# OpenDriveLab/MTGS

Measured on AMD Instinct MI355X. Metric: rendered Mpix/s (fwd+bwd) @ 2M Gaussians 1920x1080, higher is better.
Workload: dtype f32

## Files before the change

mtgs_amd/csrc/bin3.hip:

```cpp
#include "common.hpp"
#include "tile_rect.hpp"
#include "devsize.hpp"
#include "raster_rec.hpp"

namespace {

using mtgs_os::SizeRef;

constexpr int B3_BLOCK = 256;
constexpr int MAX_BINS = 32768;

struct Item { uint32_t rank, span; };
constexpr int SPAN_BITS = 12;
constexpr int MAX_ROWS = 4096;

struct RowGeom {
    int row0, h, tile0, w;
    int y0, x0;
    float mx, my, ca, cb, cc, s2max;
};
template <bool TIGHT>
__device__ __forceinline__ RowGeom row_geom(const float *__restrict__ recs, const int32_t *__restrict__ vis_ids, int64_t rank,
                                            int64_t N, int C, float ts, int tw, int th) {
    const float4 *rec = reinterpret_cast<const float4 *>(recs + rank * REC_FLOATS);
    const float4 r0 = rec[0], r1 = rec[1];
    const Rect q = tile_rect(r0.x, r0.y, __float_as_int(r1.w), ts, tw, th);
    const int cam = C == 1 ? 0 : (int)((uint32_t)vis_ids[rank] / (uint32_t)N);
    RowGeom g;
    g.row0 = cam * th + q.y0; g.h = q.y1 - q.y0; g.w = q.x1 - q.x0;
    g.tile0 = g.row0 * tw + q.x0;
    g.y0 = q.y0; g.x0 = q.x0;
    g.mx = r0.x; g.my = r0.y; g.ca = r0.z; g.cb = r0.w; g.cc = r1.x; g.s2max = r1.z;
    if (g.w <= 0) g.h = 0;
    if (TIGHT && !(g.s2max >= 0.f)) g.h = 0;
    return g;
}
template <bool TIGHT>
__device__ __forceinline__ int row_span(const RowGeom &g, int y, int tw, int &first) {
    first = g.tile0 + y * tw;
    if (!TIGHT) return g.w;
    const float a = g.ca, b = g.cb, c = g.cc, det = a * c - b * b;
    if (!(det > 0.f && a > 0.f && c > 0.f)) return g.w;
    const float ty = (float)((g.y0 + y) * MTGS_TILE_SIZE);
    const float Y0 = ty + 0.5f - g.my, Y1 = ty + 15.5f - g.my;
    const float sm = g.s2max * 1.001f + 1e-2f;
    const float rdet = 1.0f / det, ymax = sqrtf(a * sm * rdet), X = sqrtf(sm * c * rdet);
    const float yb0 = fmaxf(Y0, -ymax), yb1 = fminf(Y1, ymax);
    if (!(yb0 <= yb1)) return 0;
    const float ra = 1.0f / a, tilt = b * X / c;
    const float dyl = fminf(fmaxf(tilt, yb0), yb1), dyr = fminf(fmaxf(-tilt, yb0), yb1);
    const float xl = (-b * dyl - sqrtf(fmaxf(a * sm - det * dyl * dyl, 0.f))) * ra - 2e-3f;
    const float xr = (-b * dyr + sqrtf(fmaxf(a * sm - det * dyr * dyr, 0.f))) * ra + 2e-3f;
    const float inv = 1.0f / (float)MTGS_TILE_SIZE;
    const float fx0 = (float)g.x0, fx1 = (float)(g.x0 + g.w);
    const int lo = (int)fminf(fmaxf(ceilf((g.mx + xl - 15.5f) * inv), fx0), fx1) - g.x0;
    const int hi = (int)fmaxf(fminf(floorf((g.mx + xr - 0.5f) * inv), fx1 - 1.f), fx0 - 1.f) - g.x0 + 1;
    first += lo;
    return hi - lo;
}

__device__ __forceinline__ bool arrive_last(uint32_t *done, int64_t active, int *s_flag) {
    __syncthreads();
    if (threadIdx.x == 0)
        *s_flag = __hip_atomic_fetch_add(done, 1u, __ATOMIC_RELAXED, __HIP_MEMORY_SCOPE_AGENT) == (uint32_t)(active - 1);
    __syncthreads();
    return *s_flag != 0;
}

constexpr int R_BLOCK = 1024;
constexpr int SERIAL_MAX = 48;

struct RowShare {
    float mx[R_BLOCK], my[R_BLOCK], ca[R_BLOCK], cb[R_BLOCK], cc[R_BLOCK], s2[R_BLOCK];
    uint32_t xy[R_BLOCK];
    uint32_t wr[R_BLOCK];
    uint32_t off[R_BLOCK + 1];
    uint32_t ws[R_BLOCK / 64];
};
template <class F>
__device__ __forceinline__ void tight_rows_walk(RowShare &S, const RowGeom &g, int h, int tw, F &&emit) {
    const int tid = threadIdx.x, lane = tid & 63, wave = tid >> 6;
    S.mx[tid] = g.mx; S.my[tid] = g.my; S.ca[tid] = g.ca; S.cb[tid] = g.cb; S.cc[tid] = g.cc; S.s2[tid] = g.s2max;
    S.xy[tid] = (uint32_t)g.x0 | ((uint32_t)g.y0 << 16);
    S.wr[tid] = (uint32_t)max(g.w - 1, 0) | ((uint32_t)g.row0 << 16);
    uint32_t inc = (uint32_t)h;
#pragma unroll
    for (int o = 1; o < 64; o <<= 1) {
        const uint32_t up = __shfl_up(inc, o, 64);
        if (lane >= o) inc += up;
    }
    if (lane == 63) S.ws[wave] = inc;
    __syncthreads();
    uint32_t base = 0;
    for (int w = 0; w < wave; ++w) base += S.ws[w];
    S.off[tid] = base + inc - (uint32_t)h;
    if (tid == R_BLOCK - 1) S.off[R_BLOCK] = base + inc;
    __syncthreads();
    const uint32_t total = S.off[R_BLOCK];
    static_assert(R_BLOCK == 1 << 10, "ten bisection steps");
    for (uint32_t idx = tid; idx < total; idx += R_BLOCK) {
        int lo = 0, hi = R_BLOCK;
#pragma unroll
        for (int it = 0; it < 10; ++it) {
            const int mid = (lo + hi) >> 1;
            if (S.off[mid] <= idx) lo = mid; else hi = mid;
        }
        const int y = (int)(idx - S.off[lo]);
        RowGeom q;
        q.mx = S.mx[lo]; q.my = S.my[lo]; q.ca = S.ca[lo]; q.cb = S.cb[lo]; q.cc = S.cc[lo]; q.s2max = S.s2[lo];
        const uint32_t xy = S.xy[lo], wr = S.wr[lo];
        q.x0 = (int)(xy & 0xffffu); q.y0 = (int)(xy >> 16); q.w = (int)(wr & 0xffffu) + 1; q.row0 = (int)(wr >> 16);
        q.tile0 = q.row0 * tw + q.x0; q.h = 0;
        int first;
        const int w = row_span<true>(q, y, tw, first);
        if (w > 0) emit(lo, q.row0 + y, first, w);
    }
}
template <bool TIGHT>
__global__ __launch_bounds__(R_BLOCK) void bin3_rows_count_kernel(const SizeRef n_vis_ref, const float *__restrict__ recs,
                                                                 const int32_t *__restrict__ vis_ids, int64_t N, int C, float ts,
                                                                 int tw, int th, int n_rows, uint32_t *__restrict__ row_count,
                                                                 uint32_t *__restrict__ rbase, uint32_t *__restrict__ done,
                                                                 uint32_t *__restrict__ row_start ) {
    __shared__ uint32_t s_row[MAX_ROWS];
    __shared__ uint32_t s_ws[R_BLOCK / 64];
    __shared__ uint16_t s_tall[R_BLOCK];
    __shared__ uint32_t s_ntall;
    __shared__ int s_last;
    const int tid = threadIdx.x, lane = tid & 63, wave = tid >> 6;
    const int64_t n_vis = mtgs_os::size_of(n_vis_ref);
    const int64_t r = (int64_t)blockIdx.x * R_BLOCK + tid;
    if ((int64_t)blockIdx.x * R_BLOCK >= n_vis) {
        if (n_vis == 0 && blockIdx.x == 0)
            for (int b = tid; b <= n_rows; b += R_BLOCK) row_start[b] = 0;
        return;
    }
    for (int b = tid; b < n_rows; b += R_BLOCK) s_row[b] = 0;
    if (tid == 0) s_ntall = 0;
    __syncthreads();
    RowGeom g = {};
    int my_rows = 0;
    if (r < n_vis) {
        g = row_geom<TIGHT>(recs, vis_ids, r, N, C, ts, tw, th);
        if (g.h <= SERIAL_MAX) {
            my_rows = g.h;
            if (!TIGHT)
                for (int y = 0; y < g.h; ++y) atomicAdd(&s_row[g.row0 + y], 1u);
        } else {
            s_tall[atomicAdd(&s_ntall, 1u)] = (uint16_t)tid;
        }
    }
    if constexpr (TIGHT) {
        __shared__ RowShare s_share;
        tight_rows_walk(s_share, g, my_rows, tw, [&](int, int bin, int, int) { atomicAdd(&s_row[bin], 1u); });
    }
    __syncthreads();
    for (uint32_t q = wave; q < s_ntall; q += R_BLOCK / 64) {
        const RowGeom g = row_geom<TIGHT>(recs, vis_ids, (int64_t)blockIdx.x * R_BLOCK + s_tall[q], N, C, ts, tw, th);
        int first;
        for (int y = lane; y < g.h; y += 64)
            if (row_span<TIGHT>(g, y, tw, first) > 0) atomicAdd(&s_row[g.row0 + y], 1u);
    }
    __syncthreads();
    for (int b = tid; b < n_rows; b += R_BLOCK) {
        const uint32_t c = s_row[b];
        if (c) rbase[(size_t)blockIdx.x * n_rows + b] = __hip_atomic_fetch_add(row_count + b, c, __ATOMIC_RELAXED, __HIP_MEMORY_SCOPE_AGENT);
    }
    if (!arrive_last(done, ceil_div64(n_vis, R_BLOCK), &s_last)) return;
    constexpr int ROWS_PER_THREAD = MAX_ROWS / R_BLOCK;
    static_assert(MAX_ROWS % R_BLOCK == 0, "whole rows per thread");
    uint32_t v[ROWS_PER_THREAD], mine = 0;
#pragma unroll
    for (int e = 0; e < ROWS_PER_THREAD; ++e) {
        const int b = tid * ROWS_PER_THREAD + e;
        v[e] = b < n_rows ? mtgs_os::ld32(row_count + b) : 0u;
        mine += v[e];
    }
    uint32_t inc = mine;
#pragma unroll
    for (int o = 1; o < 64; o <<= 1) {
        const uint32_t up = __shfl_up(inc, o, 64);
        if (lane >= o) inc += up;
    }
    if (lane == 63) s_ws[wave] = inc;
    __syncthreads();
    uint32_t run = inc - mine;
    for (int w = 0; w < wave; ++w) run += s_ws[w];
#pragma unroll
    for (int e = 0; e < ROWS_PER_THREAD; ++e) {
        const int b = tid * ROWS_PER_THREAD + e;
        if (b < n_rows) row_start[b] = run;
        run += v[e];
        if (b == n_rows - 1) row_start[n_rows] = run;
    }
}

template <bool TIGHT>
__global__ __launch_bounds__(R_BLOCK) void bin3_rows_place_kernel(const SizeRef n_vis_ref, const float *__restrict__ recs,
                                                                 const int32_t *__restrict__ vis_ids, int64_t N, int C, float ts,
                                                                 int tw, int th, int n_rows, const uint32_t *__restrict__ row_start,
                                                                 const uint32_t *__restrict__ rbase, int64_t cap_items,
                                                                 Item *__restrict__ items) {
    __shared__ uint32_t s_row[MAX_ROWS];
    __shared__ uint16_t s_tall[R_BLOCK];
    __shared__ uint32_t s_ntall;
    const int tid = threadIdx.x, lane = tid & 63, wave = tid >> 6;
    const int64_t n_vis = mtgs_os::size_of(n_vis_ref);
    if ((int64_t)blockIdx.x * R_BLOCK >= n_vis) return;
    for (int b = tid; b < n_rows; b += R_BLOCK) s_row[b] = row_start[b] + rbase[(size_t)blockIdx.x * n_rows + b];
    if (tid == 0) s_ntall = 0;
    __syncthreads();
    const int64_t r = (int64_t)blockIdx.x * R_BLOCK + tid;
    RowGeom g = {};
    int my_rows = 0;
    if (r < n_vis) {
        g = row_geom<TIGHT>(recs, vis_ids, r, N, C, ts, tw, th);
        if (g.h <= SERIAL_MAX) {
            my_rows = g.h;
            if (!TIGHT)
                for (int y = 0; y < g.h; ++y) {
                    const int64_t pos = atomicAdd(&s_row[g.row0 + y], 1u);
                    if (pos < cap_items) items[pos] = Item{(uint32_t)r, ((uint32_t)(g.tile0 + y * tw) << SPAN_BITS) | (uint32_t)(g.w - 1)};
                }
        } else {
            s_tall[atomicAdd(&s_ntall, 1u)] = (uint16_t)tid;
        }
    }
    if constexpr (TIGHT) {
        __shared__ RowShare s_share;
        const int64_t r0 = (int64_t)blockIdx.x * R_BLOCK;
        tight_rows_walk(s_share, g, my_rows, tw, [&](int owner, int bin, int first, int w) {
            const int64_t pos = atomicAdd(&s_row[bin], 1u);
            if (pos < cap_items) items[pos] = Item{(uint32_t)(r0 + owner), ((uint32_t)first << SPAN_BITS) | (uint32_t)(w - 1)};
        });
    }
    __syncthreads();
    for (uint32_t q = wave; q < s_ntall; q += R_BLOCK / 64) {
        const int64_t rq = (int64_t)blockIdx.x * R_BLOCK + s_tall[q];
        const RowGeom g = row_geom<TIGHT>(recs, vis_ids, rq, N, C, ts, tw, th);
        for (int y = lane; y < g.h; y += 64) {
            int first;
            const int w = row_span<TIGHT>(g, y, tw, first);
            if (w <= 0) continue;
            const int64_t pos = atomicAdd(&s_row[g.row0 + y], 1u);
            if (pos < cap_items) items[pos] = Item{(uint32_t)rq, ((uint32_t)first << SPAN_BITS) | (uint32_t)(w - 1)};
        }
    }
}

constexpr int SM_LONG_BUCKET = 255;
constexpr int T_THREADS = 1024, T_ITEMS = 2, T_TILE = T_THREADS * T_ITEMS, SCHED_BUCKETS = 1024;
struct TileRange { int lo, hi; };
__device__ __forceinline__ TileRange tile_range(const Item *__restrict__ items, int64_t base, int64_t n_items, int tw) {
    const int64_t last = min(n_items, base + T_TILE) - 1;
    const int first_tile = (int)(items[base].span >> SPAN_BITS), last_tile = (int)(items[last].span >> SPAN_BITS);
    return TileRange{(first_tile / tw) * tw, (last_tile / tw + 1) * tw};
}

__global__ __launch_bounds__(T_THREADS) void bin3_tiles_count_kernel(
    const uint32_t *__restrict__ n_items_ptr, int64_t cap_items, const Item *__restrict__ items, int tw, int n_bins,
    int64_t cap_M, uint32_t *__restrict__ bins , uint32_t *__restrict__ done ,
    int32_t *__restrict__ offsets , int32_t *__restrict__ order ,
    uint32_t *__restrict__ n_long ) {
    extern __shared__ uint32_t s_bins[];
    __shared__ uint32_t s_aux[SCHED_BUCKETS];
    __shared__ uint32_t s_ws[T_THREADS / 64];
    __shared__ uint16_t s_wide[T_TILE];
    __shared__ uint32_t s_nwide;
    __shared__ int s_last;
    const int tid = threadIdx.x, lane = tid & 63, wave = tid >> 6;
    const int64_t n_items = min((int64_t)*n_items_ptr, cap_items);
    if ((int64_t)blockIdx.x * T_TILE >= n_items) {
        if (n_items == 0 && blockIdx.x == 0) {
            for (int b = tid; b <= n_bins; b += T_THREADS) offsets[b] = 0;
            for (int b = tid; b < n_bins; b += T_THREADS) order[b] = b;
            if (tid == 0) *n_long = 0;
        }
        return;
    }
    for (int64_t base = (int64_t)blockIdx.x * T_TILE; base < n_items; base += (int64_t)gridDim.x * T_TILE) {
        const TileRange tr = tile_range(items, base, n_items, tw);
        for (int b = tr.lo + tid; b < tr.hi; b += T_THREADS) s_bins[b] = 0;
        if (tid == 0) s_nwide = 0;
        __syncthreads();
#pragma unroll
        for (int e = 0; e < T_ITEMS; ++e) {
            const int64_t i = base + e * T_THREADS + tid;
            if (i < n_items) {
                const Item it = items[i];
                const int t0 = (int)(it.span >> SPAN_BITS), w = (int)(it.span & ((1u << SPAN_BITS) - 1)) + 1;
                if (w <= SERIAL_MAX) {
                    for (int x = 0; x < w; ++x) atomicAdd(&s_bins[t0 + x], 1u);
                } else {
                    s_wide[atomicAdd(&s_nwide, 1u)] = (uint16_t)(e * T_THREADS + tid);
                }
            }
        }
        __syncthreads();
        for (uint32_t q = wave; q < s_nwide; q += T_THREADS / 64) {
            const Item it = items[base + s_wide[q]];
            const int t0 = (int)(it.span >> SPAN_BITS), w = (int)(it.span & ((1u << SPAN_BITS) - 1)) + 1;
            for (int x = lane; x < w; x += 64) atomicAdd(&s_bins[t0 + x], 1u);
        }
        __syncthreads();
        for (int b = tr.lo + tid; b < tr.hi; b += T_THREADS) {
            const uint32_t c = s_bins[b];
            if (c) {
                const uint32_t before = __hip_atomic_fetch_add(bins + b, c, __ATOMIC_RELAXED, __HIP_MEMORY_SCOPE_AGENT);
                asm volatile("" ::"v"(before));
            }
        }
        __syncthreads();
    }
    if (!arrive_last(done, min((int64_t)gridDim.x, ceil_div64(n_items, T_TILE)), &s_last)) return;
    for (int b = tid; b < n_bins; b += T_THREADS) s_bins[b] = mtgs_os::ld32(bins + b);
    __syncthreads();
    const int per = (n_bins + T_THREADS - 1) / T_THREADS;
    const int b0 = tid * per, b1 = min(n_bins, b0 + per);
    uint32_t mine = 0;
    for (int b = b0; b < b1; ++b) mine += s_bins[b];
    uint32_t inc = mine;
#pragma unroll
    for (int o = 1; o < 64; o <<= 1) {
        const uint32_t up = __shfl_up(inc, o, 64);
        if (lane >= o) inc += up;
    }
    if (lane == 63) s_ws[wave] = inc;
    __syncthreads();
    uint32_t wb = 0;
    for (int w = 0; w < wave; ++w) wb += s_ws[w];
    uint64_t run = (uint64_t)wb + inc - mine;
    const uint64_t cap = (uint64_t)cap_M;
    for (int b = b0; b < b1; ++b) {
        const uint64_t lo = run < cap ? run : cap;
        run += s_bins[b];
        const uint64_t hi = run < cap ? run : cap;
        offsets[b] = (int32_t)lo;
        s_bins[b] = (uint32_t)(hi - lo);
        if (b == n_bins - 1) offsets[n_bins] = (int32_t)hi;
    }
    s_aux[tid] = 0;
    __syncthreads();
    auto bucket_of = [&](int t) { return SCHED_BUCKETS - 1 - min((int)(s_bins[t] >> 2), SCHED_BUCKETS - 1); };
    for (int t = tid; t < n_bins; t += T_THREADS) atomicAdd(&s_aux[bucket_of(t)], 1u);
    __syncthreads();
    const uint32_t hv = s_aux[tid];
    uint32_t hinc = hv;
#pragma unroll
    for (int o = 1; o < 64; o <<= 1) {
        const uint32_t up = __shfl_up(hinc, o, 64);
        if (lane >= o) hinc += up;
    }
    if (lane == 63) s_ws[wave] = hinc;
    __syncthreads();
    uint32_t hb = 0;
    for (int w = 0; w < wave; ++w) hb += s_ws[w];
    __syncthreads();
    s_aux[tid] = hb + hinc - hv;
    __syncthreads();
    if (tid == 0) *n_long = s_aux[SCHED_BUCKETS - SM_LONG_BUCKET];
    __syncthreads();
    for (int t = tid; t < n_bins; t += T_THREADS) order[atomicAdd(&s_aux[bucket_of(t)], 1u)] = t;
}

struct TailFill {
    int mode;
    const int64_t *totals;
    int32_t *flatten_ids;
    int64_t *isect_ids;
    int64_t sentinel_key;
    int64_t *status;
    int64_t cap_vis, cap_M;
};

__global__ __launch_bounds__(T_THREADS) void bin3_tiles_place_kernel(
    const uint32_t *__restrict__ n_items_ptr, int64_t cap_items, const Item *__restrict__ items, int tw, int n_bins,
    const int32_t *__restrict__ offsets, uint32_t *__restrict__ cursor ,
    const uint64_t *__restrict__ vis_keys, uint32_t cap_keys, uint64_t *__restrict__ keys64, const TailFill tail) {
    extern __shared__ uint32_t s_bins[];
    __shared__ uint16_t s_wide[T_TILE];
    __shared__ uint32_t s_nwide;
    const int tid = threadIdx.x, lane = tid & 63, wave = tid >> 6;
    const int64_t n_items = min((int64_t)*n_items_ptr, cap_items);
    for (int64_t base = (int64_t)blockIdx.x * T_TILE; base < n_items; base += (int64_t)gridDim.x * T_TILE) {
        const TileRange tr = tile_range(items, base, n_items, tw);
        for (int b = tr.lo + tid; b < tr.hi; b += T_THREADS) s_bins[b] = 0;
        if (tid == 0) s_nwide = 0;
        __syncthreads();
        Item it[T_ITEMS];
        int t0[T_ITEMS], w[T_ITEMS];
        uint32_t depth[T_ITEMS];
#pragma unroll
        for (int e = 0; e < T_ITEMS; ++e) {
            const int64_t i = base + e * T_THREADS + tid;
            it[e] = Item{0, 0}; t0[e] = 0; w[e] = 0; depth[e] = 0;
            if (i < n_items) {
                it[e] = items[i];
                t0[e] = (int)(it[e].span >> SPAN_BITS); w[e] = (int)(it[e].span & ((1u << SPAN_BITS) - 1)) + 1;
                depth[e] = (uint32_t)vis_keys[it[e].rank];
                if (w[e] <= SERIAL_MAX) {
                    for (int x = 0; x < w[e]; ++x) atomicAdd(&s_bins[t0[e] + x], 1u);
                } else {
                    s_wide[atomicAdd(&s_nwide, 1u)] = (uint16_t)(e * T_THREADS + tid);
                    w[e] = 0;
                }
            }
        }
        __syncthreads();
        const uint32_t n_wide = s_nwide;
        for (uint32_t q = wave; q < n_wide; q += T_THREADS / 64) {
            const Item iw = items[base + s_wide[q]];
            const int tq = (int)(iw.span >> SPAN_BITS), wq = (int)(iw.span & ((1u << SPAN_BITS) - 1)) + 1;
            for (int x = lane; x < wq; x += 64) atomicAdd(&s_bins[tq + x], 1u);
        }
        __syncthreads();
        for (int b = tr.lo + tid; b < tr.hi; b += T_THREADS) {
            const uint32_t c = s_bins[b];
            if (c) s_bins[b] = (uint32_t)offsets[b] + __hip_atomic_fetch_add(cursor + b, c, __ATOMIC_RELAXED, __HIP_MEMORY_SCOPE_AGENT);
        }
        __syncthreads();
#pragma unroll
        for (int e = 0; e < T_ITEMS; ++e) {
            const uint64_t key = ((uint64_t)depth[e] << 32) | it[e].rank;
            for (int x = 0; x < w[e]; ++x) {
                const uint32_t pos = atomicAdd(&s_bins[t0[e] + x], 1u);
                if (pos < cap_keys) keys64[pos] = key;
            }
        }
        for (uint32_t q = wave; q < n_wide; q += T_THREADS / 64) {
            const Item iw = items[base + s_wide[q]];
            const int tq = (int)(iw.span >> SPAN_BITS), wq = (int)(iw.span & ((1u << SPAN_BITS) - 1)) + 1;
            const uint64_t key = ((uint64_t)(uint32_t)vis_keys[iw.rank] << 32) | iw.rank;
            for (int x = lane; x < wq; x += 64) {
                const uint32_t pos = atomicAdd(&s_bins[tq + x], 1u);
                if (pos < cap_keys) keys64[pos] = key;
            }
        }
        __syncthreads();
    }
    if (tail.status && blockIdx.x == 0 && tid == 0) {
        const int64_t packed = *tail.totals, nv = packed >> 32, m = packed & 0xFFFFFFFFll;
        tail.status[0] = nv;
        tail.status[1] = m;
        tail.status[2] = (nv > tail.cap_vis || m > tail.cap_M) ? 1 : 0;
    }
    if (tail.mode) {
        const int64_t from = offsets[n_bins];
        int64_t to = (int64_t)cap_keys;
        if (tail.mode == 2) to = min(to, (int64_t)(*tail.totals & 0xFFFFFFFFll));
        for (int64_t i = from + (int64_t)blockIdx.x * T_THREADS + tid; i < to; i += (int64_t)gridDim.x * T_THREADS) {
            tail.flatten_ids[i] = -1;
            if (tail.isect_ids) tail.isect_ids[i] = tail.sentinel_key;
        }
    }
}

struct SortEpilogue {
    int32_t *rank_ids, *flatten_ids;
    int64_t *isect_ids;
    const int32_t *vis_ids;
    uint32_t n_tiles;
    int tile_bits;
    bool single_cam;
    uint32_t rank_max;
    __device__ __forceinline__ void store(int64_t dst, uint32_t bin, uint64_t key) const {
        const int32_t rank = (int32_t)min((uint32_t)key, rank_max);
        rank_ids[dst] = rank;
        __builtin_nontemporal_store(vis_ids[rank], flatten_ids + dst);
        if (isect_ids) {
            const int64_t cam = single_cam ? 0 : bin / n_tiles, tile = single_cam ? bin : bin % n_tiles;
            __builtin_nontemporal_store((long long)((cam << (32 + tile_bits)) | (tile << 32) | (int64_t)(key >> 32)), reinterpret_cast<long long *>(isect_ids) + dst);
        }
    }
};

constexpr uint64_t KEY_INF = 0x7ff0000000000000ull;
__host__ __device__ constexpr int swz_t(int hi4) {
    return ((hi4 & 1) ? 15 : 0) ^ ((hi4 & 2) ? 11 : 0) ^ ((hi4 & 4) ? 29 : 0) ^ ((hi4 & 8) ? 17 : 0);
}
__device__ __forceinline__ int swz(int i) {
    const int t = (int)((0x1916121d040b0f00ull >> ((i >> 2) & 0x38)) & 31);
    return i ^ t ^ ((i & 256) ? 17 : 0);
}
static_assert(swz_t(1) == 0x0f && swz_t(2) == 0x0b && swz_t(3) == 0x04 && swz_t(4) == 0x1d && swz_t(5) == 0x12 &&
              swz_t(6) == 0x16 && swz_t(7) == 0x19 && swz_t(8) == 17, "packed table");
__host__ __device__ constexpr int swz_d(int d) { return d ^ swz_t((d >> 5) & 15); }
__device__ __forceinline__ void cswap(uint64_t &a, uint64_t &b) {
    const double x = __longlong_as_double((long long)a), y = __longlong_as_double((long long)b);
    double lo, hi;
    asm("v_min_f64 %0, %1, %2" : "=v"(lo) : "v"(x), "v"(y));
    asm("v_max_f64 %0, %1, %2" : "=v"(hi) : "v"(x), "v"(y));
    a = (uint64_t)__double_as_longlong(lo); b = (uint64_t)__double_as_longlong(hi);
}
template <bool WAVE> __device__ __forceinline__ void lds_sync() {
    if constexpr (WAVE) {
        __builtin_amdgcn_fence(__ATOMIC_RELEASE, "wavefront");
        __builtin_amdgcn_wave_barrier();
        __builtin_amdgcn_fence(__ATOMIC_ACQUIRE, "wavefront");
    } else {
        __syncthreads();
    }
}

template <bool WAVE, int LOGE, int STOP>
__device__ __forceinline__ void trip(uint64_t *s, int groups, int n, int nthr, int tid, int apply) {
    constexpr int E = 1 << LOGE, SLOW = STOP >> (LOGE - 1);
    if constexpr (SLOW >= 1) {
        for (int g = tid; g < groups; g += nthr) {
            const int x = ((g & ~(SLOW - 1)) << LOGE) | (g & (SLOW - 1));
            if (x >= n) continue;
            const int px = swz(x);
            uint64_t v[E];
#pragma unroll
            for (int e = 0; e < E; ++e) v[e] = s[px ^ swz_d(e * SLOW)];
#pragma unroll
            for (int bit = E >> 1; bit >= 1; bit >>= 1)
                if (apply & bit) {
#pragma unroll
                    for (int e = 0; e < E; ++e)
                        if (!(e & bit)) cswap(v[e], v[e | bit]);
                }
#pragma unroll
            for (int e = 0; e < E; ++e) s[px ^ swz_d(e * SLOW)] = v[e];
        }
        lds_sync<WAVE>();
    }
}
template <bool WAVE, int LOGE, int H>
__device__ __forceinline__ void mirror_trip(uint64_t *s, int groups, int n, int nthr, int tid) {
    constexpr int E = 1 << LOGE, HALF = E >> 1, B = H >> (LOGE - 1);
    if constexpr (B >= 1) {
        for (int g = tid; g < groups; g += nthr) {
            const int x = ((g & ~(B - 1)) << LOGE) | (g & (B - 1));
            if (x >= n) continue;
            const int low = x & (B - 1);
            const int pl = swz(x), pu = swz(x - low + H + (B - 1 - low));
            uint64_t v[E];
#pragma unroll
            for (int f = 0; f < HALF; ++f) { v[f] = s[pl ^ swz_d(f * B)]; v[HALF + f] = s[pu ^ swz_d(f * B)]; }
#pragma unroll
            for (int f = 0; f < HALF; ++f) cswap(v[f], v[E - 1 - f]);
#pragma unroll
            for (int bit = HALF >> 1; bit >= 1; bit >>= 1) {
#pragma unroll
                for (int f = 0; f < HALF; ++f)
                    if (!(f & bit)) { cswap(v[f], v[f | bit]); cswap(v[HALF + f], v[HALF + (f | bit)]); }
            }
#pragma unroll
            for (int f = 0; f < HALF; ++f) { s[pl ^ swz_d(f * B)] = v[f]; s[pu ^ swz_d(f * B)] = v[HALF + f]; }
        }
        lds_sync<WAVE>();
    }
}
#define B3_STRIDE_SWITCH(J, CALL)                                                                                   \
    switch (J) {                                                                                                     \
        case 4: CALL(4); break; case 8: CALL(8); break; case 16: CALL(16); break; case 32: CALL(32); break;          \
        case 64: CALL(64); break; case 128: CALL(128); break; case 256: CALL(256); break; case 512: CALL(512); break; \
        case 1024: CALL(1024); break; case 2048: CALL(2048); break; case 4096: CALL(4096); break;                   \
        default: CALL(8192); break;                                                                                   \
    }

template <bool WAVE, int LOGE>
__device__ __forceinline__ void level_tail(uint64_t *s, int groups, int n, int nthr, int tid, int j) {
    constexpr int E = 1 << LOGE;
    int r = 0;
    for (int q = j; q >= 1; q >>= 1) ++r;
    while (r > LOGE) {
        const int take = r - LOGE >= LOGE ? LOGE : r - LOGE;
        const int apply = ((1 << take) - 1) << (LOGE - take);
#define B3_CALL(S) trip<WAVE, LOGE, S>(s, groups, n, nthr, tid, apply)
        B3_STRIDE_SWITCH(j, B3_CALL)
#undef B3_CALL
        j >>= take;
        r -= take;
    }
    trip<WAVE, LOGE, E / 2>(s, groups, n, nthr, tid, (1 << r) - 1);
}

template <bool WAVE, int LOGE>
__device__ __forceinline__ void bitonic_sort_e(uint64_t *s, int P, int n, int nthr, int tid) {
    constexpr int E = 1 << LOGE;
    const int groups = P >> LOGE;
    for (int g = tid; g < groups; g += nthr) {
        const int x = g << LOGE;
        if (x >= n) continue;
        const int px = swz(x);
        uint64_t v[E];
#pragma unroll
        for (int e = 0; e < E; ++e) v[e] = s[px ^ e];
#pragma unroll
        for (int k = 2; k <= E; k <<= 1) {
#pragma unroll
            for (int e = 0; e < E; ++e)
                if ((e ^ (k - 1)) > e) cswap(v[e], v[e ^ (k - 1)]);
#pragma unroll
            for (int j = k >> 2; j >= 1; j >>= 1) {
#pragma unroll
                for (int e = 0; e < E; ++e)
                    if (!(e & j)) cswap(v[e], v[e | j]);
            }
        }
#pragma unroll
        for (int e = 0; e < E; ++e) s[px ^ e] = v[e];
    }
    lds_sync<WAVE>();
    for (int k = 2 * E; k <= P; k <<= 1) {
        const int h = k >> 1;
#define B3_CALL(S) mirror_trip<WAVE, LOGE, S>(s, groups, n, nthr, tid)
        B3_STRIDE_SWITCH(h, B3_CALL)
#undef B3_CALL
        if ((k >> (LOGE + 1)) >= 1) level_tail<WAVE, LOGE>(s, groups, n, nthr, tid, k >> (LOGE + 1));
    }
}
template <bool WAVE, int P16 = 1 << 30>
__device__ __forceinline__ void bitonic_sort(uint64_t *s, int P, int n, int nthr, int tid) {
    if constexpr (P16 < (1 << 30)) {
        if (P >= P16) { bitonic_sort_e<WAVE, 4>(s, P, n, nthr, tid); return; }
    }
    bitonic_sort_e<WAVE, 3>(s, P, n, nthr, tid);
}

__device__ __forceinline__ int pow2_ceil(int n) {
    int p = 8;
    while (p < n) p <<= 1;
    return p;
}

template <bool WAVE, int P16 = 1 << 30>
__device__ __forceinline__ void sort_tile_lds(uint64_t *s, const uint64_t *__restrict__ keys, int64_t o0, int L, uint32_t bin,
                                              int nthr, int tid, const SortEpilogue &epi) {
    const int P = pow2_ceil(L);
    for (int i = tid; i < P; i += nthr) s[swz(i)] = i < L ? keys[o0 + i] : KEY_INF;
    lds_sync<WAVE>();
    bitonic_sort<WAVE, P16>(s, P, L, nthr, tid);
    for (int i = tid; i < L; i += nthr) epi.store(o0 + i, bin, s[swz(i)]);
    lds_sync<WAVE>();
}

constexpr int SM_CAP = 4096, SM_WAVE_CAP = 1024, SM_TILES = 4;
constexpr int LG_THREADS = 1024, LG_CAP = 16384;
__global__ __launch_bounds__(B3_BLOCK, 4) void bin3_sort_small_kernel(const int32_t *__restrict__ offsets,
                                                                  const int32_t *__restrict__ order, int n_bins,
                                                                  const uint32_t *__restrict__ n_long_ptr, int64_t cap_M,
                                                                  const uint64_t *__restrict__ keys, const SortEpilogue epi) {
    __shared__ uint64_t s_keys[SM_CAP];
    static_assert(SM_CAP == SM_TILES * SM_WAVE_CAP, "one buffer: a long list, or four short ones");
    const int tid = threadIdx.x, wave = tid >> 6, lane = tid & 63;
    const int n_long = (int)*n_long_ptr;
    const bool together = (int)blockIdx.x < n_long;
    const int g = together ? (int)blockIdx.x : n_long + ((int)blockIdx.x - n_long) * SM_TILES + wave;
    if (g >= n_bins) return;
    const int bin = order[g];
    const int o0 = offsets[bin], L = offsets[bin + 1] - o0;
    if (L == 0 || L > SM_CAP || (int64_t)o0 + L > cap_M) return;
    if (together) sort_tile_lds<false, 4096>(s_keys, keys, o0, L, (uint32_t)bin, B3_BLOCK, tid, epi);
    else if (L <= SM_WAVE_CAP) sort_tile_lds<true, 1024>(s_keys + wave * SM_WAVE_CAP, keys, o0, L, (uint32_t)bin, 64, lane, epi);
}

__global__ __launch_bounds__(LG_THREADS) void bin3_sort_large_kernel(const int32_t *__restrict__ offsets,
                                                                    const int32_t *__restrict__ order, int n_bins, int64_t cap_M,
                                                                    uint64_t *keys, const SortEpilogue epi) {
    extern __shared__ uint64_t s_big[];
    const int tid = threadIdx.x;
    for (int g = blockIdx.x; g < n_bins; g += gridDim.x) {
        const int bin = order[g];
        const int64_t o0 = offsets[bin];
        const int L = offsets[bin + 1] - (int)o0;
        if (L <= SM_CAP) {
            if ((L >> 2) < SCHED_BUCKETS - 1) break;
            continue;
        }
        if (o0 + L > cap_M) continue;
        if (L <= LG_CAP) {
            sort_tile_lds<false>(s_big, keys, o0, L, (uint32_t)bin, LG_THREADS, tid, epi);
            continue;
        }
        uint64_t *seg = keys + o0;
        const int nch = (L + LG_CAP - 1) / LG_CAP;
        for (int c = 0; c < nch; ++c) {
            const int c0 = c * LG_CAP, n = min(LG_CAP, L - c0);
            for (int i = tid; i < LG_CAP; i += LG_THREADS) s_big[swz(i)] = i < n ? seg[c0 + i] : KEY_INF;
            __syncthreads();
            bitonic_sort<false>(s_big, LG_CAP, n, LG_THREADS, tid);
            for (int i = tid; i < n; i += LG_THREADS) seg[c0 + i] = s_big[swz(i)];
            __syncthreads();
        }
        int64_t P = LG_CAP;
        while (P < L) P <<= 1;
        for (int64_t k = 2 * LG_CAP; k <= P; k <<= 1) {
            const int64_t half = k >> 1;
            for (int64_t i = tid; i < P / 2; i += LG_THREADS) {
                const int64_t b = (i / half) * k, o = i % half, lo = b + o, hi = b + k - 1 - o;
                if (hi < L) {
                    uint64_t a = seg[lo], z = seg[hi];
                    if (a > z) { seg[lo] = z; seg[hi] = a; }
                }
            }
            __syncthreads();
            for (int64_t j = k >> 2; j >= LG_CAP; j >>= 1) {
                for (int64_t i = tid; i < P / 2; i += LG_THREADS) {
                    const int64_t lo = (i / j) * 2 * j + i % j, hi = lo + j;
                    if (hi < L) {
                        uint64_t a = seg[lo], z = seg[hi];
                        if (a > z) { seg[lo] = z; seg[hi] = a; }
                    }
                }
                __syncthreads();
            }
            for (int c = 0; c < nch; ++c) {
                const int c0 = c * LG_CAP, n = min(LG_CAP, L - c0);
                for (int i = tid; i < LG_CAP; i += LG_THREADS) s_big[swz(i)] = i < n ? seg[c0 + i] : KEY_INF;
                __syncthreads();
                level_tail<false, 3>(s_big, LG_CAP >> 3, n, LG_THREADS, tid, LG_CAP >> 1);
                for (int i = tid; i < n; i += LG_THREADS) seg[c0 + i] = s_big[swz(i)];
                __syncthreads();
            }
        }
        for (int i = tid; i < L; i += LG_THREADS) epi.store(o0 + i, (uint32_t)bin, seg[i]);
        __syncthreads();
    }
}

inline int bit_length_u32(uint32_t v) {
    int b = 0;
    while (v) { ++b; v >>= 1; }
    return b;
}

struct Bin3Workspace {
    char *control;
    size_t control_bytes;
    uint32_t *done_rows, *done_tiles, *n_long, *row_count, *bins, *cursor;
    uint32_t *row_start, *rbase;
    int32_t *order;
    Item *items;
    uint64_t *keys64;
    size_t total;
};
inline Bin3Workspace carve3(char *base, int64_t cap_vis, int64_t cap_M, int n_rows, int n_bins) {
    Bin3Workspace w;
    size_t off = 0;
    auto take = [&](size_t bytes) { char *p = base ? base + off : nullptr; off += mtgs_os::align256(bytes); return p; };
    const int64_t m = cap_M > 0 ? cap_M : 1, nv = cap_vis > 0 ? cap_vis : 1;
    w.control = base;
    char *misc = take(64);
    w.done_rows = (uint32_t *)misc; w.done_tiles = (uint32_t *)misc + 1; w.n_long = (uint32_t *)misc + 2;
    w.row_count = (uint32_t *)take((size_t)n_rows * 4);
    w.bins = (uint32_t *)take((size_t)n_bins * 4);
    w.cursor = (uint32_t *)take((size_t)n_bins * 4);
    w.control_bytes = off;
    w.row_start = (uint32_t *)take((size_t)(n_rows + 1) * 4);
    w.rbase = (uint32_t *)take((size_t)ceil_div64(nv, R_BLOCK) * n_rows * 4);
    w.order = (int32_t *)take((size_t)n_bins * 4);
    w.items = (Item *)take((size_t)m * sizeof(Item));
    w.keys64 = (uint64_t *)take((size_t)m * 8);
    w.total = off;
    return w;
}

}

extern "C" int mtgs_bin3_supported(int C, int tile_w, int tile_h, int64_t cap_M) {
    return C > 0 && tile_w > 0 && tile_h > 0 && (int64_t)C * tile_w * tile_h <= MAX_BINS && (int64_t)C * tile_h <= MAX_ROWS && tile_w <= (1 << SPAN_BITS) &&
                   cap_M < ((int64_t)1 << 30)
               ? 1 : 0;
}

extern "C" int mtgs_bin3_control_bytes(int C, int tile_w, int tile_h, size_t *bytes) {
    MTGS_REQUIRE(C > 0 && tile_w > 0 && tile_h > 0 && bytes, MTGS_EINVAL, "mtgs_bin3_control_bytes: bad arguments");
    *bytes = carve3(nullptr, 1, 1, C * tile_h, C * tile_w * tile_h).control_bytes;
    return MTGS_OK;
}

extern "C" int mtgs_bin3_workspace_bytes(int C, int tile_w, int tile_h, int64_t cap_vis, int64_t cap_M, size_t *bytes) {
    MTGS_REQUIRE(C > 0 && tile_w > 0 && tile_h > 0 && cap_vis >= 0 && cap_M >= 0 && bytes, MTGS_EINVAL,
                 "mtgs_bin3_workspace_bytes: bad arguments");
    *bytes = carve3(nullptr, cap_vis, cap_M, C * tile_h, C * tile_w * tile_h).total;
    return MTGS_OK;
}

extern "C" int mtgs_bin3_build(int C, int64_t N, int tile_size, int tile_w, int tile_h, int64_t *totals,
                               int64_t cap_vis, int64_t cap_M, const float *recs, const int32_t *vis_ids,
                               const int64_t *vis_keys, int32_t *rank_ids,
                               int32_t *flatten_ids, int64_t *isect_ids, int32_t *offsets, int32_t *tile_order, int flags,
                               void *ws, size_t ws_bytes, void *stream) {
    const int tight = flags & MTGS_BIN3_TIGHT;
    MTGS_REQUIRE((flags & ~(MTGS_BIN3_TIGHT | MTGS_BIN3_FILL_TO_M | MTGS_BIN3_FILL_TO_CAP | MTGS_BIN3_PREZEROED | MTGS_BIN3_STATUS)) == 0, MTGS_EINVAL,
                 "mtgs_bin3_build: unknown flags %d", flags);
    MTGS_REQUIRE(C > 0 && N >= 0 && tile_w > 0 && tile_h > 0 && cap_vis >= 0 && cap_M >= 0, MTGS_EINVAL, "mtgs_bin3_build: bad sizes");
    MTGS_REQUIRE(tile_size == MTGS_TILE_SIZE, MTGS_EUNSUPPORTED, "mtgs_bin3_build: tile_size=%d (only 16 is implemented)", tile_size);
    MTGS_REQUIRE(mtgs_bin3_supported(C, tile_w, tile_h, cap_M), MTGS_EUNSUPPORTED,
                 "mtgs_bin3_build: %d x %d x %d (camera, tile) pairs / %lld intersections (at most %d pairs, %d (camera, tile row) "
                 "pairs and 2^30 intersections; use mtgs_bin_build)", C, tile_w, tile_h, (long long)cap_M, MAX_BINS, MAX_ROWS);
    MTGS_REQUIRE(totals && recs && vis_ids && vis_keys && rank_ids && flatten_ids && offsets && ws, MTGS_EINVAL,
                 "mtgs_bin3_build: null pointer");
    const int n_bins = C * tile_w * tile_h, n_rows = C * tile_h;
    MTGS_REQUIRE((reinterpret_cast<uintptr_t>(ws) & 255) == 0, MTGS_EINVAL, "mtgs_bin3_build: workspace must be 256-byte aligned");
    Bin3Workspace w = carve3((char *)ws, cap_vis, cap_M, n_rows, n_bins);
    MTGS_REQUIRE(ws_bytes >= w.total, MTGS_EWORKSPACE, "mtgs_bin3_build: workspace %zu < %zu bytes", ws_bytes, w.total);
    hipStream_t st = (hipStream_t)stream;
    if (!(flags & MTGS_BIN3_PREZEROED))
        if (int rc = mtgs_zero_async(w.control, w.control_bytes, st)) return rc;
    const SizeRef n_vis_ref{totals, 1, cap_vis};
    int32_t *order = tile_order ? tile_order : w.order;
    const unsigned r_grid = (unsigned)ceil_div64(cap_vis > 0 ? cap_vis : 1, R_BLOCK);
    const unsigned t_grid = (unsigned)min((int64_t)512, ceil_div64(cap_M > 0 ? cap_M : 1, T_TILE));
    const float ts = (float)tile_size;
    if (tight) {
        bin3_rows_count_kernel<true><<<r_grid, R_BLOCK, 0, st>>>(n_vis_ref, recs, vis_ids, N, C, ts, tile_w, tile_h, n_rows, w.row_count,
                                                                w.rbase, w.done_rows, w.row_start);
        bin3_rows_place_kernel<true><<<r_grid, R_BLOCK, 0, st>>>(n_vis_ref, recs, vis_ids, N, C, ts, tile_w, tile_h, n_rows, w.row_start,
                                                                w.rbase, cap_M, w.items);
    } else {
        bin3_rows_count_kernel<false><<<r_grid, R_BLOCK, 0, st>>>(n_vis_ref, recs, vis_ids, N, C, ts, tile_w, tile_h, n_rows, w.row_count,
                                                                 w.rbase, w.done_rows, w.row_start);
        bin3_rows_place_kernel<false><<<r_grid, R_BLOCK, 0, st>>>(n_vis_ref, recs, vis_ids, N, C, ts, tile_w, tile_h, n_rows, w.row_start,
                                                                 w.rbase, cap_M, w.items);
    }
    const int tile_bits_ = bit_length_u32((uint32_t)(tile_w * tile_h));
    const TailFill tail{cap_M > 0 ? ((flags & MTGS_BIN3_FILL_TO_CAP) ? 4 : ((flags & MTGS_BIN3_FILL_TO_M) ? 2 : 0)) : 0, totals, flatten_ids, isect_ids,
                        ((int64_t)(C - 1) << (32 + tile_bits_)) | ((int64_t)(tile_w * tile_h - 1) << 32) | (int64_t)0x7f800000,
                        (flags & MTGS_BIN3_STATUS) ? totals + 1 : nullptr, cap_vis, cap_M};
    bin3_tiles_count_kernel<<<t_grid, T_THREADS, (size_t)n_bins * 4, st>>>(w.row_start + n_rows, cap_M, w.items, tile_w, n_bins,
                                                                            cap_M, w.bins, w.done_tiles, offsets, order, w.n_long);
    bin3_tiles_place_kernel<<<t_grid, T_THREADS, (size_t)n_bins * 4, st>>>(w.row_start + n_rows, cap_M, w.items, tile_w, n_bins,
                                                                            offsets, w.cursor, (const uint64_t *)vis_keys, (uint32_t)(cap_M > 0 ? cap_M : 1), w.keys64, tail);
    const SortEpilogue epi{rank_ids, flatten_ids, isect_ids, vis_ids, (uint32_t)(tile_w * tile_h),
                           bit_length_u32((uint32_t)(tile_w * tile_h)), C == 1, (uint32_t)(cap_vis > 0 ? cap_vis - 1 : 0)};
    static const bool big_lds = [] {
        return hipFuncSetAttribute((const void *)bin3_sort_large_kernel, hipFuncAttributeMaxDynamicSharedMemorySize,
                                   LG_CAP * 8) == hipSuccess &&
               hipFuncSetAttribute((const void *)bin3_tiles_place_kernel, hipFuncAttributeMaxDynamicSharedMemorySize,
                                   MAX_BINS * 4) == hipSuccess &&
               hipFuncSetAttribute((const void *)bin3_tiles_count_kernel, hipFuncAttributeMaxDynamicSharedMemorySize,
                                   MAX_BINS * 4) == hipSuccess;
    }();
    MTGS_REQUIRE(big_lds, MTGS_ELAUNCH, "mtgs_bin3_build: cannot reserve %d bytes of LDS per workgroup", LG_CAP * 8);
    bin3_sort_large_kernel<<<(unsigned)min(n_bins, 256), LG_THREADS, (size_t)LG_CAP * 8, st>>>(
        offsets, order, n_bins, cap_M, w.keys64, epi);
    bin3_sort_small_kernel<<<(unsigned)n_bins, B3_BLOCK, 0, st>>>(offsets, order, n_bins, w.n_long, cap_M, w.keys64, epi);
    MTGS_CHECK_LAUNCH("mtgs_bin3_build");
    return MTGS_OK;
}
```

Before: 2643.

## Move tile scan out of count kernel; placers compute offsets locally

The count kernel no longer elects a last-arriving block to prefix-scan all bins and build the tile schedule. Block 0 of the place kernel now builds the schedule (offsets, order, long-bin count) while the other blocks derive each bin's start offset themselves by summing the global bin counts before and inside their tile range. This removes the serial last-block tail and the done counter from the count kernel and overlaps scheduling with placement. In exchange every placer block re-reads the bin counts (redundant global reads), and an explicit waves-per-EU occupancy hint is added to the place kernel.

```diff
diff --git a/mtgs_amd/csrc/bin3.hip b/mtgs_amd/csrc/bin3.hip
--- a/mtgs_amd/csrc/bin3.hip
+++ b/mtgs_amd/csrc/bin3.hip
@@ -258,26 +258,13 @@
 }
 
 __global__ __launch_bounds__(T_THREADS) void bin3_tiles_count_kernel(
-    const uint32_t *__restrict__ n_items_ptr, int64_t cap_items, const Item *__restrict__ items, int tw, int n_bins,
-    int64_t cap_M, uint32_t *__restrict__ bins , uint32_t *__restrict__ done ,
-    int32_t *__restrict__ offsets , int32_t *__restrict__ order ,
-    uint32_t *__restrict__ n_long ) {
+    const uint32_t *__restrict__ n_items_ptr, int64_t cap_items, const Item *__restrict__ items, int tw,
+    uint32_t *__restrict__ bins ) {
     extern __shared__ uint32_t s_bins[];
-    __shared__ uint32_t s_aux[SCHED_BUCKETS];
-    __shared__ uint32_t s_ws[T_THREADS / 64];
     __shared__ uint16_t s_wide[T_TILE];
     __shared__ uint32_t s_nwide;
-    __shared__ int s_last;
     const int tid = threadIdx.x, lane = tid & 63, wave = tid >> 6;
     const int64_t n_items = min((int64_t)*n_items_ptr, cap_items);
-    if ((int64_t)blockIdx.x * T_TILE >= n_items) {
-        if (n_items == 0 && blockIdx.x == 0) {
-            for (int b = tid; b <= n_bins; b += T_THREADS) offsets[b] = 0;
-            for (int b = tid; b < n_bins; b += T_THREADS) order[b] = b;
-            if (tid == 0) *n_long = 0;
-        }
-        return;
-    }
     for (int64_t base = (int64_t)blockIdx.x * T_TILE; base < n_items; base += (int64_t)gridDim.x * T_TILE) {
         const TileRange tr = tile_range(items, base, n_items, tw);
         for (int b = tr.lo + tid; b < tr.hi; b += T_THREADS) s_bins[b] = 0;
@@ -305,15 +292,40 @@
         __syncthreads();
         for (int b = tr.lo + tid; b < tr.hi; b += T_THREADS) {
             const uint32_t c = s_bins[b];
-            if (c) {
-                const uint32_t before = __hip_atomic_fetch_add(bins + b, c, __ATOMIC_RELAXED, __HIP_MEMORY_SCOPE_AGENT);
-                asm volatile("" ::"v"(before));
-            }
-        }
-        __syncthreads();
-    }
-    if (!arrive_last(done, min((int64_t)gridDim.x, ceil_div64(n_items, T_TILE)), &s_last)) return;
-    for (int b = tid; b < n_bins; b += T_THREADS) s_bins[b] = mtgs_os::ld32(bins + b);
+            if (c) __hip_atomic_fetch_add(bins + b, c, __ATOMIC_RELAXED, __HIP_MEMORY_SCOPE_AGENT);
+        }
+        __syncthreads();
+    }
+}
+
+struct TailFill {
+    int mode;
+    const int64_t *totals;
+    int32_t *flatten_ids;
+    int64_t *isect_ids;
+    int64_t sentinel_key;
+    int64_t *status;
+    int64_t cap_vis, cap_M;
+};
+
+__device__ __forceinline__ uint32_t wave_sum_u32(uint32_t v) {
+#pragma unroll
+    for (int o = 32; o >= 1; o >>= 1) v += __shfl_xor(v, o, 64);
+    return v;
+}
+
+__device__ __forceinline__ void tile_schedule(const uint32_t *__restrict__ bins, int n_bins, bool empty, int64_t cap_M,
+                                              int32_t *__restrict__ offsets , int32_t *__restrict__ order ,
+                                              uint32_t *__restrict__ n_long ,
+                                              uint32_t *s_bins, uint32_t *s_aux, uint32_t *s_ws) {
+    const int tid = threadIdx.x, lane = tid & 63, wave = tid >> 6;
+    if (empty) {
+        for (int b = tid; b <= n_bins; b += T_THREADS) offsets[b] = 0;
+        for (int b = tid; b < n_bins; b += T_THREADS) order[b] = b;
+        if (tid == 0) *n_long = 0;
+        return;
+    }
+    for (int b = tid; b < n_bins; b += T_THREADS) s_bins[b] = bins[b];
     __syncthreads();
     const int per = (n_bins + T_THREADS - 1) / T_THREADS;
     const int b0 = tid * per, b1 = min(n_bins, b0 + per);
@@ -363,28 +375,37 @@
     for (int t = tid; t < n_bins; t += T_THREADS) order[atomicAdd(&s_aux[bucket_of(t)], 1u)] = t;
 }
 
-struct TailFill {
-    int mode;
-    const int64_t *totals;
-    int32_t *flatten_ids;
-    int64_t *isect_ids;
-    int64_t sentinel_key;
-    int64_t *status;
-    int64_t cap_vis, cap_M;
-};
-
-__global__ __launch_bounds__(T_THREADS) void bin3_tiles_place_kernel(
+__global__ __launch_bounds__(T_THREADS) __attribute__((amdgpu_waves_per_eu(8, 8))) void bin3_tiles_place_kernel(
     const uint32_t *__restrict__ n_items_ptr, int64_t cap_items, const Item *__restrict__ items, int tw, int n_bins,
-    const int32_t *__restrict__ offsets, uint32_t *__restrict__ cursor ,
-    const uint64_t *__restrict__ vis_keys, uint32_t cap_keys, uint64_t *__restrict__ keys64, const TailFill tail) {
+    const uint32_t *__restrict__ bins, uint32_t *__restrict__ cursor , int32_t *__restrict__ offsets, int32_t *__restrict__ order,
+    uint32_t *__restrict__ n_long, const uint64_t *__restrict__ vis_keys, uint32_t cap_keys, uint64_t *__restrict__ keys64,
+    const TailFill tail) {
     extern __shared__ uint32_t s_bins[];
     __shared__ uint16_t s_wide[T_TILE];
+    __shared__ uint32_t s_aux[SCHED_BUCKETS];
+    __shared__ uint32_t s_ws[T_THREADS / 64], s_wf[T_THREADS / 64];
     __shared__ uint32_t s_nwide;
     const int tid = threadIdx.x, lane = tid & 63, wave = tid >> 6;
     const int64_t n_items = min((int64_t)*n_items_ptr, cap_items);
-    for (int64_t base = (int64_t)blockIdx.x * T_TILE; base < n_items; base += (int64_t)gridDim.x * T_TILE) {
+    const uint64_t cap = (uint64_t)tail.cap_M;
+    if (blockIdx.x == 0) tile_schedule(bins, n_bins, n_items == 0, tail.cap_M, offsets, order, n_long, s_bins, s_aux, s_ws);
+    const int64_t placers = (int64_t)gridDim.x - 1;
+    for (int64_t base = blockIdx.x == 0 ? n_items : ((int64_t)blockIdx.x - 1) * T_TILE; base < n_items; base += placers * T_TILE) {
         const TileRange tr = tile_range(items, base, n_items, tw);
         for (int b = tr.lo + tid; b < tr.hi; b += T_THREADS) s_bins[b] = 0;
+        const int per = (tr.hi - tr.lo + T_THREADS - 1) / T_THREADS;
+        const int b0 = min(tr.hi, tr.lo + tid * per), b1 = min(tr.hi, b0 + per);
+        uint32_t front = 0, mine = 0;
+        for (int b = tid; b < tr.lo; b += T_THREADS) front += bins[b];
+        for (int b = b0; b < b1; ++b) mine += bins[b];
+        uint32_t inc = mine;
+#pragma unroll
+        for (int o = 1; o < 64; o <<= 1) {
+            const uint32_t up = __shfl_up(inc, o, 64);
+            if (lane >= o) inc += up;
+        }
+        front = wave_sum_u32(front);
+        if (lane == 63) { s_ws[wave] = inc; s_wf[wave] = front; }
         if (tid == 0) s_nwide = 0;
         __syncthreads();
         Item it[T_ITEMS];
@@ -414,9 +435,12 @@
             for (int x = lane; x < wq; x += 64) atomicAdd(&s_bins[tq + x], 1u);
         }
         __syncthreads();
-        for (int b = tr.lo + tid; b < tr.hi; b += T_THREADS) {
+        uint64_t run = inc - mine;
+        for (int wv = 0; wv < T_THREADS / 64; ++wv) run += (uint64_t)s_wf[wv] + (wv < wave ? s_ws[wv] : 0u);
+        for (int b = b0; b < b1; ++b) {
             const uint32_t c = s_bins[b];
-            if (c) s_bins[b] = (uint32_t)offsets[b] + __hip_atomic_fetch_add(cursor + b, c, __ATOMIC_RELAXED, __HIP_MEMORY_SCOPE_AGENT);
+            if (c) s_bins[b] = (uint32_t)(run < cap ? run : cap) + __hip_atomic_fetch_add(cursor + b, c, __ATOMIC_RELAXED, __HIP_MEMORY_SCOPE_AGENT);
+            run += bins[b];
         }
         __syncthreads();
 #pragma unroll
@@ -445,7 +469,14 @@
         tail.status[2] = (nv > tail.cap_vis || m > tail.cap_M) ? 1 : 0;
     }
     if (tail.mode) {
-        const int64_t from = offsets[n_bins];
+        uint32_t part = 0;
+        for (int b = tid; b < n_bins; b += T_THREADS) part += bins[b];
+        part = wave_sum_u32(part);
+        if (lane == 0) s_wf[wave] = part;
+        __syncthreads();
+        uint64_t listed = 0;
+        for (int w = 0; w < T_THREADS / 64; ++w) listed += s_wf[w];
+        const int64_t from = (int64_t)(listed < cap ? listed : cap);
         int64_t to = (int64_t)cap_keys;
         if (tail.mode == 2) to = min(to, (int64_t)(*tail.totals & 0xFFFFFFFFll));
         for (int64_t i = from + (int64_t)blockIdx.x * T_THREADS + tid; i < to; i += (int64_t)gridDim.x * T_THREADS) {
@@ -730,7 +761,7 @@
 struct Bin3Workspace {
     char *control;
     size_t control_bytes;
-    uint32_t *done_rows, *done_tiles, *n_long, *row_count, *bins, *cursor;
+    uint32_t *done_rows, *n_long, *row_count, *bins, *cursor;
     uint32_t *row_start, *rbase;
     int32_t *order;
     Item *items;
@@ -744,7 +775,7 @@
     const int64_t m = cap_M > 0 ? cap_M : 1, nv = cap_vis > 0 ? cap_vis : 1;
     w.control = base;
     char *misc = take(64);
-    w.done_rows = (uint32_t *)misc; w.done_tiles = (uint32_t *)misc + 1; w.n_long = (uint32_t *)misc + 2;
+    w.done_rows = (uint32_t *)misc; w.n_long = (uint32_t *)misc + 1;
     w.row_count = (uint32_t *)take((size_t)n_rows * 4);
     w.bins = (uint32_t *)take((size_t)n_bins * 4);
     w.cursor = (uint32_t *)take((size_t)n_bins * 4);
@@ -821,10 +852,11 @@
     const TailFill tail{cap_M > 0 ? ((flags & MTGS_BIN3_FILL_TO_CAP) ? 4 : ((flags & MTGS_BIN3_FILL_TO_M) ? 2 : 0)) : 0, totals, flatten_ids, isect_ids,
                         ((int64_t)(C - 1) << (32 + tile_bits_)) | ((int64_t)(tile_w * tile_h - 1) << 32) | (int64_t)0x7f800000,
                         (flags & MTGS_BIN3_STATUS) ? totals + 1 : nullptr, cap_vis, cap_M};
-    bin3_tiles_count_kernel<<<t_grid, T_THREADS, (size_t)n_bins * 4, st>>>(w.row_start + n_rows, cap_M, w.items, tile_w, n_bins,
-                                                                            cap_M, w.bins, w.done_tiles, offsets, order, w.n_long);
-    bin3_tiles_place_kernel<<<t_grid, T_THREADS, (size_t)n_bins * 4, st>>>(w.row_start + n_rows, cap_M, w.items, tile_w, n_bins,
-                                                                            offsets, w.cursor, (const uint64_t *)vis_keys, (uint32_t)(cap_M > 0 ? cap_M : 1), w.keys64, tail);
+    bin3_tiles_count_kernel<<<t_grid, T_THREADS, (size_t)n_bins * 4, st>>>(w.row_start + n_rows, cap_M, w.items, tile_w, w.bins);
+    const unsigned p_grid = (unsigned)min((int64_t)511, ceil_div64(cap_M > 0 ? cap_M : 1, T_TILE));
+    bin3_tiles_place_kernel<<<p_grid + 1, T_THREADS, (size_t)n_bins * 4, st>>>(w.row_start + n_rows, cap_M, w.items, tile_w, n_bins, w.bins, w.cursor,
+                                                                                offsets, order, w.n_long, (const uint64_t *)vis_keys,
+                                                                                (uint32_t)(cap_M > 0 ? cap_M : 1), w.keys64, tail);
     const SortEpilogue epi{rank_ids, flatten_ids, isect_ids, vis_ids, (uint32_t)(tile_w * tile_h),
                            bit_length_u32((uint32_t)(tile_w * tile_h)), C == 1, (uint32_t)(cap_vis > 0 ? cap_vis - 1 : 0)};
     static const bool big_lds = [] {
```

New measurement: 2669, median of 6. No clear change (+1.0%).
